# VGLoic/kzg-poly-commit-exploration

Hardware: AMD Instinct MI355X
Metric: g1_msm_commitments_per_sec_degree_2^20 (higher is better)
Workload: dtype i32 digits (Fp: 13 signed radix-2^30 digits, Montgomery 2^390; Fr: 8 x u32, Montgomery 2^256)

## Files before the change

kzg_poly_commit_exploration_amd/csrc/api.hip:

```cpp
#include <hip/hip_runtime.h>
#include <sys/random.h>

#include <algorithm>
#include <atomic>
#include <cerrno>
#include <chrono>
#include <condition_variable>
#include <cstdio>
#include <cstdlib>
#include <cstring>
#include <deque>
#include <functional>
#include <mutex>
#include <new>
#include <string>
#include <thread>
#include <vector>

#include "../../include/kzg_mi355x.h"
#include "engine.h"
#include "host_field.hpp"
#include "host_fr.hpp"
#include "fr30_host.hpp"
#include "host_pairing.hpp"
#include "host_sha256.hpp"
#include "wire30.hip.h"

using namespace kzg;
namespace hf = kzg_host;

namespace {

constexpr size_t kMaxCoefficients = 0xFFFFFFFFull;

#ifndef KZG_NUM_SLOTS
#define KZG_NUM_SLOTS 5
#endif
constexpr int kNumSlots = KZG_NUM_SLOTS;
struct ReducePlan {
    uint32_t lo_bits = 0, hi_bits = 0;
    uint32_t row_lo = 0, row_hi = 0;
    uint32_t col_lo = 0, col_hi = 0;
    uint32_t off_r2row = 0, off_c2row = 0, off_r2col = 0, off_c2col = 0, total = 0;
};

enum SlotKind { SLOT_IDLE = 0, SLOT_COMMIT = 1, SLOT_OPEN = 2, SLOT_TRIVIAL = 3, SLOT_COMMIT_BATCH = 4, SLOT_OPEN_BATCH = 5, SLOT_RESERVED = 6,
                SLOT_OPEN_POINTS = 7 ,
                SLOT_OPEN_COMBINED = 8 ,
                SLOT_OPEN_SETS = 9  };

int hip_fail(kzg_ctx* ctx, const char* what, hipError_t e);

struct DevBuf {
    void* p = nullptr;
    size_t cap = 0;
    DevBuf() = default;
    DevBuf(const DevBuf&) = delete;
    DevBuf& operator=(const DevBuf&) = delete;
    ~DevBuf() { reset(); }
    void reset() {
        if (p) hipFree(p);
        p = nullptr;
        cap = 0;
    }
    template <class T = uint32_t> T* dev() const { return (T*)p; }
    int reserve(kzg_ctx* ctx, size_t bytes, hipStream_t drain = nullptr) { return bytes <= cap ? KZG_OK : grow(ctx, bytes, drain); }
    int grow(kzg_ctx* ctx, size_t bytes, hipStream_t drain) {
        if (drain)
            if (hipError_t e = hipStreamSynchronize(drain)) return hip_fail(ctx, "hipStreamSynchronize", e);
        reset();
        if (hipError_t e = hipMalloc(&p, bytes)) {
            p = nullptr;
            return hip_fail(ctx, "hipMalloc", e);
        }
        cap = bytes;
        return KZG_OK;
    }
};
struct PinnedBuf {
    enum Kind { Mapped, Staged };
    const Kind kind;
    void *h = nullptr, *d = nullptr;
    size_t cap = 0;
    explicit PinnedBuf(Kind k) : kind(k) {}
    PinnedBuf(const PinnedBuf&) = delete;
    PinnedBuf& operator=(const PinnedBuf&) = delete;
    ~PinnedBuf() { reset(); }
    void reset() {
        if (h) hipHostFree(h);
        if (d && kind == Staged) hipFree(d);
        h = d = nullptr;
        cap = 0;
    }
    template <class T = uint32_t> T* host() const { return (T*)h; }
    template <class T = uint32_t> T* dev() const { return (T*)d; }
    int reserve(kzg_ctx* ctx, size_t bytes, hipStream_t drain = nullptr) { return bytes <= cap ? KZG_OK : grow(ctx, bytes, drain); }
    int grow(kzg_ctx* ctx, size_t bytes, hipStream_t drain) {
        if (drain)
            if (hipError_t e = hipStreamSynchronize(drain)) return hip_fail(ctx, "hipStreamSynchronize", e);
        reset();
        hipError_t e = hipHostMalloc(&h, bytes, kind == Mapped ? hipHostMallocMapped : hipHostMallocDefault);
        if (e == hipSuccess) e = kind == Mapped ? hipHostGetDevicePointer(&d, h, 0) : hipMalloc(&d, bytes);
        if (e != hipSuccess) {
            d = nullptr;
            reset();
            return hip_fail(ctx, kind == Mapped ? "hipHostMalloc (mapped)" : "hipHostMalloc + hipMalloc (staging)", e);
        }
        cap = bytes;
        return KZG_OK;
    }
};
template <int N>
struct Workspace {
    DevBuf buf[N];
    int get(kzg_ctx* ctx, int i, size_t bytes, void** out) {
        DevBuf& b = buf[i];
        int rc = KZG_OK;
        if (!bytes && !b.p) {
            rc = b.reserve(ctx, 256);
            b.cap = 0;
        } else {
            rc = b.reserve(ctx, bytes);
        }
        *out = b.p;
        return rc;
    }
};

struct SlotQueue {
    hipStream_t stream = nullptr;
    hipStream_t end = nullptr;
    hipEvent_t ev[8] = {};
    hipEvent_t done = nullptr;
    hipEvent_t sorted_ev = nullptr, accum_ev = nullptr;
    hipEvent_t cmb_ev[2] = {};
    hipEvent_t cells_ev = nullptr;
    hipEvent_t upload_ev = nullptr;
    SlotQueue() = default;
    SlotQueue(const SlotQueue&) = delete;
    SlotQueue& operator=(const SlotQueue&) = delete;
    ~SlotQueue() {
        for (hipEvent_t e : {ev[0], ev[1], ev[2], ev[3], ev[4], ev[5], ev[6], ev[7], cmb_ev[0], cmb_ev[1], cells_ev, upload_ev, done, sorted_ev, accum_ev})
            if (e) hipEventDestroy(e);
    }
};

struct Slot : SlotQueue {
    DevBuf cnt, offs, block_sums, pairs, sorted, buckets;
    DevBuf recoded;
    DevBuf part_a, part_b;
    DevBuf pair_scratch;
    DevBuf heavy_ws;
    DevBuf arena;
    PinnedBuf fin{PinnedBuf::Mapped};
    DevBuf stage;
    DevBuf q;
    DevBuf chunk, block;
    PinnedBuf small{PinnedBuf::Mapped};
    PinnedBuf bsmall{PinnedBuf::Mapped};
    std::vector<uint32_t> open_ys;
    PinnedBuf roots{PinnedBuf::Staged};
    PinnedBuf pvals{PinnedBuf::Mapped};
    DevBuf pblock;
    std::vector<uint32_t> pts_ys;
    size_t pts_nq = 0;
    PinnedBuf ctab{PinnedBuf::Staged};
    PinnedBuf cvals{PinnedBuf::Mapped};
    DevBuf cpart, cin;
    size_t cmb_t = 0;
    float combine_ms = 0;
    PinnedBuf stab{PinnedBuf::Staged}, ssel{PinnedBuf::Staged};
    PinnedBuf svals{PinnedBuf::Mapped};
    DevBuf sg;
    std::vector<uint32_t> sets_vmap;
    PinnedBuf ltab{PinnedBuf::Staged};
    DevBuf lag_part;
    DevBuf gp_in, gp_z, gp_part;
    PinnedBuf gp_flags{PinnedBuf::Mapped};
    DevBuf cpoly, cagg;
    SlotKind kind = SLOT_IDLE;
    size_t job_n = 0;
    uint32_t job_batch = 1;
    uint32_t open_y[8] = {};
    bool timing = false;
    bool has_quotient = false;
    bool tail_checked = false;
    kzg_kernel_times times = {};
};

}

struct kzg_ctx {
    kzg::MultiState* multi = nullptr;
    int device = 0;
    std::mutex mu;
    std::condition_variable slot_cv;
    int sync_owned = 0;
    bool raw_partials = false;
    bool host_trace = false;
    std::atomic<uint64_t> trace_ns[5] = {};
    std::atomic<uint64_t> trace_calls{0};
    std::string last_error;
    size_t n = 0;
    MsmConfig cfg = {};
    DevBuf table;
    DevBuf ntt_tw;
    DevBuf lag_table;
    size_t lag_n = 0;
    uint64_t srs_gen = 0;
    ReducePlan plan;
    size_t arena_records = 0, final_records = 0;
    uint32_t max_batch = 1;
    Slot slots[kNumSlots];
    hipStream_t front_stream = nullptr, heavy_stream = nullptr, tail_stream = nullptr;
    hipStream_t upload_stream = nullptr;
    uint32_t accum_lds_bytes = 41u * 1024u;
    uint32_t small_lds_bytes = 48u * 1024u;
    bool small_msm_off = false;
    bool slots_ready = false;
    bool timing = false;
    std::mutex fk20_mu;
    DevBuf glv;
    uint32_t glv_log = 0;
    DevBuf fk20_B, fk20_tab;
    uint32_t fk20_log_L = 0, fk20_log_l = 0;
    Workspace<11> fk20_ws;
    std::mutex recover_mu;
    DevBuf rec_g;
    Workspace<11> rec_ws;
    Workspace<17> vc_ws;
    Workspace<8> blob_ws;
    std::mutex lookup_mu;
    Workspace<6> lu_ws;
    std::mutex quotient_mu;
    Workspace<11> pq_ws;
    uint32_t pq_zinv_key = ~0u;
    std::vector<kzg_circuit*> circuits;
};

struct kzg_circuit {
    kzg_ctx* owner = nullptr;
    uint32_t lg_n = 0, lg_ext = 0;
    size_t n = 0, t = 0;
    uint64_t shifts[4 * kPqMaxColumns] = {};
    DevBuf values;
    DevBuf coeffs;
    DevBuf coset;
    DevBuf l0;
    DevBuf zinv;
    size_t N() const { return n << lg_ext; }
    size_t cols() const { return 2 * t + 2; }
};

namespace {

#define HIP_TRY(ctx, expr)                                                                          \
    do {                                                                                            \
        hipError_t _e = (expr);                                                                     \
        if (_e != hipSuccess) {                                                                     \
            (ctx)->last_error = std::string(#expr) + ": " + hipGetErrorString(_e);                  \
            return KZG_ERR_HIP;                                                                     \
        }                                                                                           \
    } while (0)

int hip_fail(kzg_ctx* ctx, const char* what, hipError_t e) {
// ... 47 lines not shown
    if (!ctx->upload_stream) HIP_TRY(ctx, hipStreamCreateWithFlags(&ctx->upload_stream, hipStreamNonBlocking));
    for (auto& e : s.ev)
        if (!e) HIP_TRY(ctx, hipEventCreate(&e));
    if (!s.upload_ev) HIP_TRY(ctx, hipEventCreateWithFlags(&s.upload_ev, hipEventDisableTiming));
    s.stream = s.end = ctx->front_stream;
    if (!s.done) HIP_TRY(ctx, hipEventCreateWithFlags(&s.done, hipEventDisableTiming));
    return s.small.reserve(ctx, 64 * 4);
}

int upload_unlocked(kzg_ctx* ctx, std::unique_lock<std::mutex>& lk, Slot& s, void* dst, const void* src, size_t bytes) {
    if (!bytes) return KZG_OK;
    int rc = copy_unlocked(ctx, lk, ctx->upload_stream, dst, src, bytes, hipMemcpyHostToDevice, kCopyCoeffs);
    if (rc) return rc;
    HIP_TRY(ctx, hipEventRecord(s.upload_ev, ctx->upload_stream));
    HIP_TRY(ctx, hipStreamWaitEvent(s.stream, s.upload_ev, 0));
    return KZG_OK;
}

int ensure_poly(kzg_ctx* ctx, Slot& s, size_t n) {
    const size_t cap = n < 1024 ? 1024 : n;
    if (cap * 32 <= s.stage.cap) return KZG_OK;
    if (s.done) HIP_TRY(ctx, hipEventSynchronize(s.done));
    HIP_TRY(ctx, hipStreamSynchronize(ctx->upload_stream));
    HIP_TRY(ctx, hipStreamSynchronize(s.stream));
    for (DevBuf* b : {&s.stage, &s.q, &s.chunk, &s.block}) b->reset();
    int rc = s.stage.reserve(ctx, cap * 32);
    if (rc == KZG_OK) rc = s.q.reserve(ctx, cap * 32);
    if (rc == KZG_OK) rc = s.chunk.reserve(ctx, poly_chunk_words((uint32_t)cap) * 4);
    if (rc == KZG_OK) rc = s.block.reserve(ctx, poly_block_words((uint32_t)cap) * 4);
    if (rc) s.stage.reset();
    return rc;
}

void plan_reduce(kzg_ctx* ctx) {
    ReducePlan P;
    uint32_t bits = 0;
    while ((1u << bits) < ctx->cfg.nb) bits++;
    P.lo_bits = bits / 2;
    P.hi_bits = bits - P.lo_bits;
    P.row_lo = P.hi_bits / 2;
    P.row_hi = P.hi_bits - P.row_lo;
    P.col_lo = P.lo_bits / 2;
    P.col_hi = P.lo_bits - P.col_lo;
    P.off_r2row = 0;
    P.off_c2row = P.off_r2row + (1u << P.row_hi);
    P.off_r2col = P.off_c2row + (1u << P.row_lo);
    P.off_c2col = P.off_r2col + (1u << P.col_hi);
    P.total = P.off_c2col + (1u << P.col_lo);
    ctx->plan = P;
    ctx->arena_records = ((size_t)1 << P.hi_bits) + ((size_t)1 << P.lo_bits);
    ctx->final_records = P.total;
}

int setup_slots_impl(kzg_ctx* ctx);
int setup_slots(kzg_ctx* ctx, bool keep_table_on_failure = false) {
    ctx->slots_ready = false;
    int rc = setup_slots_impl(ctx);
    if (rc != KZG_OK) {
        for (auto& s : ctx->slots) free_slot_msm(s);
        if (keep_table_on_failure) return rc;
        ctx->table.reset();
        ctx->lag_table.reset();
        ctx->lag_n = 0;
        ctx->n = 0;
        (void)hipGetLastError();
    }
    return rc;
}
int setup_slots_impl(kzg_ctx* ctx) {
    plan_reduce(ctx);
    if (const char* v = std::getenv("KZG_TEST_FAIL_SLOT_ALLOC")) {
        const int mode = std::atoi(v);
        if (mode == 1 || (mode == 2 && ctx->max_batch > 1)) {
            ctx->last_error = "injected allocation failure (KZG_TEST_FAIL_SLOT_ALLOC)";
            return KZG_ERR_HIP;
        }
    }
    if (!ctx->heavy_stream) {
        int rc = create_stream(ctx, &ctx->heavy_stream, true);
        if (rc) return rc;
    }
    if (!ctx->tail_stream) {
        int rc = create_stream(ctx, &ctx->tail_stream, false);
        if (rc) return rc;
    }
    const MsmConfig cfg = ctx->cfg;
    if (ctx->max_batch > sort_max_batch(cfg)) ctx->max_batch = sort_max_batch(cfg);
    const size_t B = ctx->max_batch;
    const size_t pairs = (size_t)cfg.max_digits * ctx->n * B;
    for (int i = 0; i < kNumSlots; i++) {
        Slot& s = ctx->slots[i];
        {
            int rcb = ensure_slot_basics(ctx, s);
            if (rcb) return rcb;
        }
        if (!s.sorted_ev) {
            HIP_TRY(ctx, hipEventCreateWithFlags(&s.sorted_ev, hipEventDisableTiming));
            HIP_TRY(ctx, hipEventCreateWithFlags(&s.accum_ev, hipEventDisableTiming));
        }
        free_slot_msm(s);
        int rc = s.cnt.reserve(ctx, (size_t)sort_count_entries((uint32_t)B, cfg) * 4 + 64);
        if (rc == KZG_OK) rc = s.offs.reserve(ctx, ((size_t)cfg.nb * B + 1) * 4);
        if (rc == KZG_OK) rc = s.block_sums.reserve(ctx, (size_t)sort_workspace_words() * 4);
        if (rc) return rc;
        HIP_TRY(ctx, hipMemset(s.block_sums.p, 0, (size_t)sort_workspace_zero_words() * 4));
        rc = s.pairs.reserve(ctx, (pairs ? pairs : 1) * 8);
        if (rc == KZG_OK) rc = s.recoded.reserve(ctx, (ctx->n * B ? ctx->n * B : 1) * 32);
        if (rc == KZG_OK) rc = s.sorted.reserve(ctx, (pairs ? pairs : 1) * 4);
        if (rc == KZG_OK) rc = s.buckets.reserve(ctx, (size_t)cfg.nb * B * kXyzzBytes);
        if (rc == KZG_OK) rc = s.part_a.reserve(ctx, (size_t)kMaxAccumLanes * kXyzzBytes);
        if (rc == KZG_OK) rc = s.part_b.reserve(ctx, (size_t)kMaxAccumLanes * kXyzzBytes);
        if (rc == KZG_OK) rc = s.pair_scratch.reserve(ctx, accumulate_pair_scratch_bytes(pairs));
        if (rc == KZG_OK) rc = s.heavy_ws.reserve(ctx, heavy_workspace_bytes());
        if (rc == KZG_OK) rc = s.arena.reserve(ctx, ctx->arena_records * B * kXyzzBytes);
        if (rc == KZG_OK) rc = s.fin.reserve(ctx, ctx->final_records * B * kXyzzBytes);
        if (rc) return rc;
        s.kind = SLOT_IDLE;
    }
    ctx->slots_ready = true;
    return KZG_OK;
}

int build_tables(kzg_ctx* ctx, hipStream_t st, void* d_xyzz_tmp, void* d_prefix) {
    const size_t n = ctx->n;
    for (uint32_t j = 1; j < ctx->cfg.W; j++) {
        char* prev = (char*)ctx->table.p + (size_t)(j - 1) * n * kAffineBytes;
        char* next = (char*)ctx->table.p + (size_t)j * n * kAffineBytes;
        launch_table_window(st, prev, (uint32_t)n, ctx->cfg.level_bits, d_xyzz_tmp, d_prefix, next);
    }
    HIP_TRY(ctx, hipGetLastError());
    HIP_TRY(ctx, hipStreamSynchronize(st));
    return KZG_OK;
}

int drain_all(kzg_ctx* ctx) {
    for (hipStream_t st : {ctx->upload_stream, ctx->front_stream, ctx->heavy_stream, ctx->tail_stream})
        if (st) HIP_TRY(ctx, hipStreamSynchronize(st));
    return KZG_OK;
}

static int srs_release(kzg_ctx* ctx) {
    ctx->slots_ready = false;
    int rc = drain_all(ctx);
    if (rc) return rc;
    for (auto& s : ctx->slots) s.kind = SLOT_IDLE;
    ctx->table.reset();
    ctx->fk20_B.reset();
    ctx->fk20_tab.reset();
    ctx->lag_table.reset();
    ctx->lag_n = 0;
    ctx->srs_gen++;
    ctx->n = 0;
    return KZG_OK;
}

int srs_prepare(kzg_ctx* ctx, size_t n) {
    if (n == 0 || n > 0x7fffffffu / 32) return KZG_ERR_INVALID_ARG;
    int rc = srs_release(ctx);
    if (rc) return rc;
    size_t free_b = 0, total_b = 0;
    HIP_TRY(ctx, hipMemGetInfo(&free_b, &total_b));
    size_t budget = (size_t)((double)free_b * 0.6);
    if (const char* v = std::getenv("KZG_TABLE_GB")) budget = (size_t)(std::strtod(v, nullptr) * 1073741824.0);
    MsmConfig cfg = choose_msm_config(n, budget);
    if ((size_t)cfg.W * n >= 0x80000000ull) return KZG_ERR_INVALID_ARG;
    ctx->cfg = cfg;
    return ctx->table.reserve(ctx, (size_t)cfg.W * n * kAffineBytes);
}

struct MsmBasis {
    const void* table;
    uint32_t stride;
};
int enqueue_msm(kzg_ctx* ctx, Slot& s, const uint32_t* d_scalars, int is_mont, size_t n, int ev_base,
                uint32_t batch = 1, uint64_t stride = 0, const MsmBasis* basis = nullptr) {
    const MsmConfig cfg = ctx->cfg;
    const void* table = basis ? basis->table : ctx->table.p;
    const uint32_t table_stride = basis ? basis->stride : (uint32_t)ctx->n;
    const uint32_t nbt = cfg.nb * batch;
    hipStream_t st = s.stream;
    s.end = st;
    if (s.timing) HIP_TRY(ctx, hipEventRecord(s.ev[ev_base], st));
    const bool header_zeroed = launch_bucket_sort(st, d_scalars, is_mont, (uint32_t)n, batch, stride, table_stride, cfg, s.cnt.dev(),
                       s.block_sums.dev(), s.pairs.dev<uint64_t>(), s.recoded.dev(), s.offs.dev(), s.sorted.dev(), (uint32_t*)s.heavy_ws.p);
    if (s.timing) {
        HIP_TRY(ctx, hipEventRecord(s.ev[ev_base + 1], st));
        HIP_TRY(ctx, hipEventRecord(s.ev[ev_base + 2], st));
    }
    bool alone = true;
    for (const auto& other : ctx->slots) alone = alone && (&other == &s || other.kind == SLOT_IDLE);
    const uint64_t max_refs = (uint64_t)n * cfg.max_digits * batch;
    const uint32_t lanes = accumulate_lanes(max_refs, alone);
    const ReducePlan& P = ctx->plan;
    const uint32_t R = 1u << P.hi_bits, C = 1u << P.lo_bits, B = batch;
    char* row = (char*)s.arena.p;
    char* col = row + (size_t)R * B * kXyzzBytes;
    char* fin = (char*)s.fin.d;
    const uint32_t rl = 1u << P.row_lo, rh = 1u << P.row_hi, cl = 1u << P.col_lo, ch = 1u << P.col_hi;
    const TreeSumDesc stage1[2] = {
        {s.buckets.p, row, B * R, C, C, 1, B * R, 0},
        {s.buckets.p, col, B * C, R, 1, C, C, (uint64_t)cfg.nb}};
    const TreeSumDesc stage2[4] = {
        {row, fin + (size_t)P.off_r2row * B * kXyzzBytes, B * rh, rl, rl, 1, rh, R},
        {row, fin + (size_t)P.off_c2row * B * kXyzzBytes, B * rl, rh, 1, rl, rl, R},
        {col, fin + (size_t)P.off_r2col * B * kXyzzBytes, B * ch, cl, cl, 1, ch, C},
        {col, fin + (size_t)P.off_c2col * B * kXyzzBytes, B * cl, ch, 1, cl, cl, C}};
    if (!header_zeroed) HIP_TRY(ctx, hipMemsetAsync(s.heavy_ws.p, 0, kHeavyHeaderBytes, st));
    if (max_refs <= kTinyRefs && !ctx->small_msm_off) {
        if (s.timing) HIP_TRY(ctx, hipEventRecord(s.ev[ev_base + 3], st));
        launch_small_msm(st, table, s.sorted.dev(), s.offs.dev(), nbt, lanes, max_refs, s.buckets.p, s.part_a.p, s.part_b.p,
                         s.heavy_ws.p, s.small.dev() + 26, stage1, stage2, ctx->small_lds_bytes);
        if (s.timing) HIP_TRY(ctx, hipEventRecord(s.ev[ev_base + 4], st));
    } else {
        const bool hand_over = !alone;
        hipStream_t hs = hand_over ? ctx->heavy_stream : st;
        if (hand_over) {
            HIP_TRY(ctx, hipEventRecord(s.sorted_ev, st));
            HIP_TRY(ctx, hipStreamWaitEvent(hs, s.sorted_ev, 0));
        }
        if (s.timing) HIP_TRY(ctx, hipEventRecord(s.ev[ev_base + 3], hs));
        launch_bucket_accumulate(hs, table, s.sorted.dev(), s.offs.dev(), nbt, lanes, s.buckets.p, s.part_a.p, s.part_b.p,
                                 ctx->accum_lds_bytes, s.pair_scratch.p, max_refs,
                                 (char*)s.heavy_ws.p + kAccumClockOffset);
        if (s.timing) HIP_TRY(ctx, hipEventRecord(s.ev[ev_base + 4], hs));
        if (hand_over) {
            HIP_TRY(ctx, hipEventRecord(s.accum_ev, hs));
            st = s.end = ctx->tail_stream;
            HIP_TRY(ctx, hipStreamWaitEvent(st, s.accum_ev, 0));
        }
        launch_bucket_finalize(st, s.offs.dev(), nbt, lanes, s.part_a.p, s.part_b.p, s.buckets.p, s.heavy_ws.p, s.small.dev() + 26,
                               finalize_group_size(nbt));
        launch_tree_sums_two_stage(st, stage1, 2, stage2, 4, (uint32_t*)s.heavy_ws.p + 64, alone);
    }
    if (s.timing) HIP_TRY(ctx, hipEventRecord(s.ev[ev_base + 5], st));
    HIP_TRY(ctx, hipGetLastError());
    return KZG_OK;
}

hf::PX host_wsum(const uint64_t* recs, uint32_t len) {
    hf::PX run = hf::px_inf(), acc = hf::px_inf();
    for (uint32_t v = len; v-- > 1;) {
        run = hf::px_add(run, hf::px_from_record(recs + (size_t)v * kXyzzWords64));
        acc = hf::px_add(acc, run);
    }
    return acc;
}
hf::PX host_shift(hf::PX p, uint32_t k) {
    for (uint32_t i = 0; i < k; i++) p = hf::px_double(p);
    return p;
}
hf::P1 finish_msm(const kzg_ctx* ctx, const Slot& s, uint32_t p = 0, uint32_t batch = 1) {
    const ReducePlan& P = ctx->plan;
    const uint64_t* f = s.fin.host<uint64_t>();
    auto at = [&](uint32_t off, uint32_t len) { return f + ((size_t)off * batch + (size_t)p * len) * kXyzzWords64; };
    const uint32_t rh = 1u << P.row_hi, rl = 1u << P.row_lo, ch = 1u << P.col_hi, cl = 1u << P.col_lo;
    hf::PX w_row = hf::px_add(host_shift(host_wsum(at(P.off_r2row, rh), rh), P.row_lo), host_wsum(at(P.off_c2row, rl), rl));
    hf::PX w_col = hf::px_add(host_shift(host_wsum(at(P.off_r2col, ch), ch), P.col_lo), host_wsum(at(P.off_c2col, cl), cl));
    hf::PX total = hf::px_add(host_shift(w_row, P.lo_bits), w_col);
    if (ctx->cfg.recode == kRecodeNaf) total = hf::px_double(total);
    const uint64_t* r2 = at(P.off_r2row, rh);
    for (uint32_t k = 0; k < rh; k++) total = hf::px_add(total, hf::px_from_record(r2 + (size_t)k * kXyzzWords64));
    return ctx->raw_partials ? hf::px_to_jacobian(total) : hf::px_normalize(total);
}

void write_p1(uint64_t out[18], const hf::P1& p) { std::memcpy(out, &p, sizeof p); }

void fill_device_times(Slot& s) {
    s.times.references = s.small.host()[26];
    const uint64_t not_start = (uint64_t)s.small.host()[28] | ((uint64_t)s.small.host()[29] << 32);
    const uint64_t end = (uint64_t)s.small.host()[30] | ((uint64_t)s.small.host()[31] << 32);
    if (not_start != 0 && end > ~not_start) s.times.accumulate_ms = (float)((double)(end - ~not_start) * 1e-5);
}
void fill_accumulate_times(Slot& s) {
    float ms = 0;
    (void)hipEventElapsedTime(&ms, s.ev[3], s.ev[4]);
    s.times.accumulate_events_ms = ms;
    if (s.times.accumulate_ms == 0) s.times.accumulate_ms = ms;
}

void slot_idle(kzg_ctx* ctx, Slot& s) {
    s.kind = SLOT_IDLE;
    ctx->slot_cv.notify_all();
}
int reserve_slot(kzg_ctx* ctx, std::unique_lock<std::mutex>& lk, bool block) {
    for (;;) {
        for (int i = 0; i < kNumSlots; i++)
            if (ctx->slots[i].kind == SLOT_IDLE) {
                ctx->slots[i].kind = SLOT_RESERVED;
                ctx->sync_owned++;
                return i;
            }
        if (!block || ctx->sync_owned == 0) return -1;
        ctx->slot_cv.wait(lk);
    }
}
void release_owned(kzg_ctx* ctx, int slot) {
    if (ctx->slots[slot].kind == SLOT_RESERVED) ctx->slots[slot].kind = SLOT_IDLE;
    ctx->sync_owned--;
    ctx->slot_cv.notify_all();
}
struct SlotLease {
    kzg_ctx* ctx;
    int slot;
    ~SlotLease() { if (slot >= 0) release_owned(ctx, slot); }
};
void quiesce(kzg_ctx* ctx, std::unique_lock<std::mutex>& lk) {
    while (ctx->sync_owned > 0) ctx->slot_cv.wait(lk);
}

bool host_tail_nonzero(const uint64_t* coeffs, size_t from, size_t n) {
    for (size_t i = from; i < n; i++)
        if (coeffs[4 * i] | coeffs[4 * i + 1] | coeffs[4 * i + 2] | coeffs[4 * i + 3]) return true;
    return false;
}

int points_weights(kzg_ctx* ctx, const uint64_t* zs, size_t k, uint64_t* ws ) {
    if (k < 1 || k > KZG_MAX_OPEN_POINTS) {
        ctx->last_error = "multiproof: k must be in [1, KZG_MAX_OPEN_POINTS]";
        return KZG_ERR_INVALID_ARG;
    }
// ... 60 lines not shown
    switch (status) {
        case KZG_OK: return "ok";
        case KZG_ERR_DEGREE_TOO_HIGH:
            return "Setup does not allow for commitment generation of the polynomial. The polynomial degree is too high.";
        case KZG_ERR_CONSTANT_POLY: return "Unable to divide a constant polynomial";
        case KZG_ERR_REMAINDER:
            return "[divide_by_root] Fail to divide the polynomial by a root, constant terms do not add up";
        case KZG_ERR_INVALID_ARG: return "invalid argument";
        case KZG_ERR_NO_DEVICE: return "no HIP device available (this library has no CPU path)";
        case KZG_ERR_HIP: return "HIP runtime error";
        case KZG_ERR_NO_SRS: return "no SRS loaded";
        case KZG_ERR_BUSY: return "slot busy";
        default: return "unknown status";
    }
}

const char* kzg_last_error(const kzg_ctx* ctx) {
    if (!ctx) return "";
    if (ctx->multi && ctx->last_error.empty()) return multi_last_error(ctx->multi);
    return ctx->last_error.c_str();
}

int kzg_ctx_create_multi_ex(const int* devices, int ndev, unsigned flags, kzg_ctx** out) {
    if (!out) return KZG_ERR_INVALID_ARG;
    *out = nullptr;
    if (!devices || ndev <= 0 || (flags & ~(unsigned)KZG_MULTI_REPLICATE_SRS)) return KZG_ERR_INVALID_ARG;
    kzg::MultiState* m = nullptr;
    std::string err;
    int rc = multi_create(devices, ndev, (flags & KZG_MULTI_REPLICATE_SRS) ? kMultiReplicate : kMultiRange, &m, err);
    if (rc != KZG_OK) return rc;
    kzg_ctx* ctx = new kzg_ctx();
    ctx->multi = m;
    ctx->device = devices[0];
    *out = ctx;
    return KZG_OK;
}
int kzg_ctx_create_multi(const int* devices, int ndev, kzg_ctx** out) { return kzg_ctx_create_multi_ex(devices, ndev, 0u, out); }
int kzg_abi_version(void) { return KZG_ABI_VERSION; }
int kzg_num_devices(const kzg_ctx* ctx) { return !ctx ? 0 : (ctx->multi ? multi_num_devices(ctx->multi) : 1); }
uint64_t kzg_rccl_exchanges(const kzg_ctx* ctx) { return (ctx && ctx->multi) ? multi_rccl_exchanges(ctx->multi) : 0; }

int kzg_ctx_create(int device, kzg_ctx** out) {
    if (!out) return KZG_ERR_INVALID_ARG;
    *out = nullptr;
    int count = 0;
    if (hipGetDeviceCount(&count) != hipSuccess || count <= 0) return KZG_ERR_NO_DEVICE;
    if (device < 0 || device >= count) return KZG_ERR_NO_DEVICE;
    if (hipSetDevice(device) != hipSuccess) return KZG_ERR_NO_DEVICE;
    kzg_ctx* ctx = new kzg_ctx();
    ctx->device = device;
    if (const char* v = std::getenv("KZG_ACCUM_LDS_KB")) ctx->accum_lds_bytes = (uint32_t)std::atoi(v) * 1024u;
    if (const char* v = std::getenv("KZG_SMALL_MSM")) ctx->small_msm_off = std::atoi(v) == 0;
    if (const char* v = std::getenv("KZG_HOST_TRACE")) ctx->host_trace = std::atoi(v) != 0;
    if (hipFuncSetAttribute(small_msm_kernel(), hipFuncAttributeMaxDynamicSharedMemorySize, (int)small_msm_lds_bytes()) == hipSuccess)
        ctx->small_lds_bytes = small_msm_lds_bytes();
    else
        (void)hipGetLastError();
    if (!poly_prepare_device() || !points_prepare_device() || !sets_prepare_device()) {
        delete ctx;
        return KZG_ERR_HIP;
    }
    *out = ctx;
    return KZG_OK;
}

void kzg_ctx_destroy(kzg_ctx* ctx) {
    if (!ctx) return;
    if (ctx->multi) {
        multi_destroy(ctx->multi);
        delete ctx;
        return;
    }
    hipSetDevice(ctx->device);
    if (ctx->host_trace && ctx->trace_calls.load()) {
        const double k = 1e-3 / (double)ctx->trace_calls.load();
        std::fprintf(stderr, "[kzg host trace] %llu kzg_commit calls, us per call: wait-for-slot %.1f upload %.1f submit %.1f device %.1f collect %.1f\n",
                     (unsigned long long)ctx->trace_calls.load(), k * ctx->trace_ns[0].load(), k * ctx->trace_ns[1].load(),
                     k * ctx->trace_ns[2].load(), k * ctx->trace_ns[3].load(), k * ctx->trace_ns[4].load());
    }
    for (hipStream_t st : {ctx->upload_stream, ctx->front_stream, ctx->heavy_stream, ctx->tail_stream})
        if (st) hipStreamSynchronize(st);
    for (hipStream_t st : {ctx->upload_stream, ctx->front_stream, ctx->heavy_stream, ctx->tail_stream})
        if (st) hipStreamDestroy(st);
    for (kzg_circuit* c : ctx->circuits) delete c;
    delete ctx;
}

size_t kzg_srs_len(const kzg_ctx* ctx) { return !ctx ? 0 : (ctx->multi ? multi_srs_len(ctx->multi) : ctx->n); }
int kzg_num_slots(const kzg_ctx*) { return kNumSlots; }

int kzg_msm_config(const kzg_ctx* ctx, int* digit_bits, int* table_levels, size_t* num_buckets, int* recoding) {
    if (ctx && ctx->multi)
        return kzg_msm_config(multi_kid(ctx->multi, 0), digit_bits, table_levels, num_buckets, recoding);
    if (!ctx || !ctx->n) return KZG_ERR_NO_SRS;
    if (digit_bits) *digit_bits = (int)ctx->cfg.c;
    if (table_levels) *table_levels = (int)ctx->cfg.W;
    if (num_buckets) *num_buckets = ctx->cfg.nb;
    if (recoding) *recoding = (int)ctx->cfg.recode;
    return KZG_OK;
}

int kzg_srs_load_g1(kzg_ctx* ctx, const void* first_g1, size_t stride, size_t n) {
    if (!ctx || !first_g1 || stride < 144) return KZG_ERR_INVALID_ARG;
    if (ctx->multi) {
        std::lock_guard<std::mutex> lkm(ctx->mu);
        ctx->last_error.clear();
// ... 509 lines not shown
        const std::string why = ctx->last_error;
        ctx->max_batch = previous;
        (void)hipGetLastError();
        (void)setup_slots(ctx);
        ctx->last_error = why;
    }
    return rc;
}

size_t kzg_max_batch(const kzg_ctx* ctx) {
    if (ctx && ctx->multi) return kzg_max_batch(multi_kid(ctx->multi, 0));
    return ctx ? ctx->max_batch : 0;
}

static int commit_batch_submit_locked(kzg_ctx* ctx, int slot, const void* d_coeffs, size_t n, size_t batch,
                                      size_t stride_coeffs, bool owned = false, bool lagrange = false) {
    if (!ctx->n || !ctx->slots_ready) return KZG_ERR_NO_SRS;
    MsmBasis basis{};
    if (lagrange && !lagrange_basis(ctx, n, &basis)) return KZG_ERR_NO_SRS;
    if (slot < 0 || slot >= kNumSlots || batch > ctx->max_batch) return KZG_ERR_INVALID_ARG;
    if (n > ctx->n) return KZG_ERR_DEGREE_TOO_HIGH;
    Slot& s = ctx->slots[slot];
    if (s.kind != (owned ? SLOT_RESERVED : SLOT_IDLE)) return KZG_ERR_BUSY;
    HIP_TRY(ctx, hipSetDevice(ctx->device));
    s.timing = ctx->timing;
    s.end = s.stream;
    s.has_quotient = false;
    s.job_n = n;
    s.job_batch = (uint32_t)batch;
    s.tail_checked = true;
    std::memset(&s.times, 0, sizeof s.times);
    std::memset(s.small.host(), 0, 64 * 4);
    int rc = enqueue_msm(ctx, s, (const uint32_t*)d_coeffs, 1, n, 0, (uint32_t)batch, stride_coeffs, lagrange ? &basis : nullptr);
    if (rc) return rc;
    HIP_TRY(ctx, hipEventRecord(s.done, s.end));
    s.kind = SLOT_COMMIT_BATCH;
    return KZG_OK;
}

int kzg_commit_batch_submit(kzg_ctx* ctx, int slot, const void* d_coeffs, size_t n, size_t batch,
                            size_t stride_coeffs) {
    KZG_SINGLE_DEVICE_ONLY(ctx);
    if (!ctx || !d_coeffs || n == 0 || batch == 0 || stride_coeffs < n || n > kMaxCoefficients) return KZG_ERR_INVALID_ARG;
    std::lock_guard<std::mutex> lk(ctx->mu);
    return commit_batch_submit_locked(ctx, slot, d_coeffs, n, batch, stride_coeffs);
}

static int wait_batch_locked(kzg_ctx* ctx, int slot, uint64_t* out_p1s, size_t batch, size_t out_stride = 18) {
    if (slot < 0 || slot >= kNumSlots) return KZG_ERR_INVALID_ARG;
    Slot& s = ctx->slots[slot];
    if (s.kind != SLOT_COMMIT_BATCH || s.job_batch != batch) return KZG_ERR_INVALID_ARG;
    HIP_TRY(ctx, hipSetDevice(ctx->device));
    slot_idle(ctx, s);
    HIP_TRY(ctx, hipEventSynchronize(s.done));
    fill_device_times(s);
    if (s.timing) {
        float ms = 0;
        (void)hipEventElapsedTime(&ms, s.ev[0], s.ev[1]); s.times.digits_ms = ms;
        (void)hipEventElapsedTime(&ms, s.ev[2], s.ev[3]); s.times.scatter_ms = ms;
        fill_accumulate_times(s);
        (void)hipEventElapsedTime(&ms, s.ev[4], s.ev[5]); s.times.reduce_ms = ms;
        (void)hipEventElapsedTime(&ms, s.ev[0], s.ev[5]); s.times.total_ms = ms;
    }
    const uint32_t B = s.job_batch;
    const uint32_t nthreads = B <= 2 ? 1 : (B < 8 ? B : 8);
    auto work = [&](uint32_t t) {
        for (uint32_t p = t; p < B; p += nthreads) write_p1(out_p1s + out_stride * (size_t)p, finish_msm(ctx, s, p, B));
    };
    if (nthreads <= 1) {
        work(0);
    } else {
        std::vector<std::thread> pool;
        for (uint32_t t = 1; t < nthreads; t++) pool.emplace_back(work, t);
        work(0);
        for (auto& th : pool) th.join();
    }
    return KZG_OK;
}

int kzg_wait_batch(kzg_ctx* ctx, int slot, uint64_t* out_p1s, size_t batch) {
    KZG_SINGLE_DEVICE_ONLY(ctx);
    if (!ctx || !out_p1s) return KZG_ERR_INVALID_ARG;
    std::lock_guard<std::mutex> lk(ctx->mu);
    return wait_batch_locked(ctx, slot, out_p1s, batch);
}

static int open_batch_submit_locked(kzg_ctx* ctx, int slot, const void* d_coeffs, size_t n, size_t batch, size_t stride_coeffs,
                                    const uint64_t* zs, const uint64_t* ys, bool owned = false) {
    if (!ctx->n || !ctx->slots_ready) return KZG_ERR_NO_SRS;
    if (slot < 0 || slot >= kNumSlots || batch > ctx->max_batch) return KZG_ERR_INVALID_ARG;
    if (n - 1 > ctx->n) return KZG_ERR_DEGREE_TOO_HIGH;
    Slot& s = ctx->slots[slot];
    if (s.kind != (owned ? SLOT_RESERVED : SLOT_IDLE)) return KZG_ERR_BUSY;
    HIP_TRY(ctx, hipSetDevice(ctx->device));
    int rc = owned ? KZG_OK : ensure_poly(ctx, s, n * batch);
    if (rc == KZG_OK) rc = s.bsmall.reserve(ctx, batch * 32 * 4, s.stream);
    if (rc) return rc;
    s.timing = ctx->timing;
    s.end = s.stream;
    s.job_n = n;
    s.job_batch = (uint32_t)batch;
    s.has_quotient = true;
    s.tail_checked = true;
    s.open_ys.assign((const uint32_t*)ys, (const uint32_t*)ys + 8 * batch);
    std::memset(&s.times, 0, sizeof s.times);
    std::memset(s.small.host(), 0, 64 * 4);
    std::memset(s.bsmall.host(), 0, batch * 32 * 4);
    if (s.timing) HIP_TRY(ctx, hipEventRecord(s.ev[6], s.stream));
    const size_t nq = n - 1;
    for (size_t p = 0; p < batch; p++) {
        const uint32_t* cp = (const uint32_t*)d_coeffs + p * stride_coeffs * 8;
        uint32_t zw[8];
        std::memcpy(zw, zs + 4 * p, 32);
        uint32_t* sm = s.bsmall.dev() + p * 32;
        PolyScratch sc{s.chunk.dev(), s.block.dev(), sm, sm + 8};
        launch_quotient(s.stream, cp, (uint32_t)n, zw, s.q.dev() + p * nq * 8, sc);
    }
    if (s.timing) HIP_TRY(ctx, hipEventRecord(s.ev[7], s.stream));
    rc = enqueue_msm(ctx, s, s.q.dev(), 1, nq, 0, (uint32_t)batch, nq);
    if (rc) return rc;
    HIP_TRY(ctx, hipEventRecord(s.done, s.end));
    s.kind = SLOT_OPEN_BATCH;
    return KZG_OK;
}

int kzg_open_batch_submit(kzg_ctx* ctx, int slot, const void* d_coeffs, size_t n, size_t batch, size_t stride_coeffs,
                          const uint64_t* zs, const uint64_t* ys) {
    KZG_SINGLE_DEVICE_ONLY(ctx);
    if (!ctx || !d_coeffs || !zs || !ys || n < 2 || batch == 0 || stride_coeffs < n || n > kMaxCoefficients) return KZG_ERR_INVALID_ARG;
    std::lock_guard<std::mutex> lk(ctx->mu);
    return open_batch_submit_locked(ctx, slot, d_coeffs, n, batch, stride_coeffs, zs, ys);
}

static int wait_open_batch_locked(kzg_ctx* ctx, int slot, uint64_t* out_p1s, int* statuses, size_t batch, size_t out_stride = 18,
                                  size_t status_stride = 1) {
    if (slot < 0 || slot >= kNumSlots) return KZG_ERR_INVALID_ARG;
    Slot& s = ctx->slots[slot];
    if (s.kind != SLOT_OPEN_BATCH || s.job_batch != batch || s.open_ys.size() != 8 * batch)
        return KZG_ERR_INVALID_ARG;
    HIP_TRY(ctx, hipSetDevice(ctx->device));
    slot_idle(ctx, s);
    HIP_TRY(ctx, hipEventSynchronize(s.done));
    fill_device_times(s);
    if (s.timing) {
        float ms = 0;
        (void)hipEventElapsedTime(&ms, s.ev[6], s.ev[7]); s.times.quotient_ms = ms;
        (void)hipEventElapsedTime(&ms, s.ev[0], s.ev[1]); s.times.digits_ms = ms;
        fill_accumulate_times(s);
        (void)hipEventElapsedTime(&ms, s.ev[4], s.ev[5]); s.times.reduce_ms = ms;
        (void)hipEventElapsedTime(&ms, s.ev[6], s.ev[5]); s.times.total_ms = ms;
    }
    const uint32_t B = s.job_batch;
    const hf::P1 inf = hf::p1_inf();
    for (uint32_t p = 0; p < B; p++) {
        const uint32_t* hs = s.bsmall.host() + p * 32;
        const uint32_t* y = s.open_ys.data() + 8 * p;
        uint64_t* out = out_p1s + out_stride * (size_t)p;
        int& status = statuses[status_stride * (size_t)p];
        if (!(hs[0] & 1u)) {
            if (std::memcmp(hs + 16, y, 32) != 0) status = KZG_ERR_CONSTANT_POLY;
            else { status = KZG_OK; write_p1(out, inf); }
            continue;
        }
        if (std::memcmp(hs + 8, y, 32) != 0) { status = KZG_ERR_REMAINDER; continue; }
        status = KZG_OK;
        write_p1(out, finish_msm(ctx, s, p, B));
    }
    s.open_ys.clear();
    return KZG_OK;
}

int kzg_wait_open_batch(kzg_ctx* ctx, int slot, uint64_t* out_p1s, int* statuses, size_t batch) {
    KZG_SINGLE_DEVICE_ONLY(ctx);
    if (!ctx || !out_p1s || !statuses) return KZG_ERR_INVALID_ARG;
    std::lock_guard<std::mutex> lk(ctx->mu);
    return wait_open_batch_locked(ctx, slot, out_p1s, statuses, batch);
}

int kzg_wait(kzg_ctx* ctx, int slot, uint64_t out_p1[18]) {
    KZG_SINGLE_DEVICE_ONLY(ctx);
    if (!ctx || !out_p1) return KZG_ERR_INVALID_ARG;
    std::lock_guard<std::mutex> lk(ctx->mu);
    return wait_locked(ctx, slot, out_p1);
}


static void await_unlocked(std::unique_lock<std::mutex>& lk, Slot& s) {
    if (s.kind == SLOT_TRIVIAL || s.kind == SLOT_RESERVED || s.kind == SLOT_IDLE) return;
    lk.unlock();
    (void)hipEventSynchronize(s.done);
    lk.lock();
}

struct HostTrace {
    kzg_ctx* ctx;
    std::chrono::steady_clock::time_point t;
    explicit HostTrace(kzg_ctx* c) : ctx(c) { if (c->host_trace) t = std::chrono::steady_clock::now(); }
    void mark(int phase) {
        if (!ctx->host_trace) return;
        const auto now = std::chrono::steady_clock::now();
        ctx->trace_ns[phase] += (uint64_t)std::chrono::duration_cast<std::chrono::nanoseconds>(now - t).count();
        t = now;
    }
};

static int commit_host(kzg_ctx* ctx, const void* scalars, int is_mont, size_t n, uint64_t out_p1[18]) {
    if (!ctx || !out_p1 || (!scalars && n)) return KZG_ERR_INVALID_ARG;
    if (n > kMaxCoefficients) return KZG_ERR_INVALID_ARG;
    if (ctx->multi) return multi_commit(ctx->multi, scalars, is_mont, n, out_p1);
    HostTrace tr(ctx);
    std::unique_lock<std::mutex> lk(ctx->mu);
    if (!ctx->n || !ctx->slots_ready) return KZG_ERR_NO_SRS;
    HIP_TRY(ctx, hipSetDevice(ctx->device));
    if (n > ctx->n && host_tail_nonzero((const uint64_t*)scalars, ctx->n, n)) return KZG_ERR_DEGREE_TOO_HIGH;
    const int slot = reserve_slot(ctx, lk, true);
    if (slot < 0) return KZG_ERR_BUSY;
    Slot& s = ctx->slots[slot];
    const size_t n_dev = n < ctx->n ? n : ctx->n;
    int rc = ensure_poly(ctx, s, n_dev);
    tr.mark(0);
// ... 6287 lines not shown
```

Before: 439.8.

## Split large batched MSMs into per-polynomial pipelined sort/accumulate/reduce stages

For batched commitments whose per-polynomial reference count exceeds a threshold, each polynomial is sorted, accumulated and reduced as its own sub-job. The sub-jobs run across the front, heavy and tail streams with per-polynomial events, so one polynomial's sort can overlap another's accumulation and reduction. The host finishes each result as soon as its tail event fires instead of waiting for the whole batch. This costs extra workspace (per-polynomial heavy workspaces and up to four sets of partial buffers), more events and launches, and per-polynomial finalize launches.

```diff
diff --git a/kzg_poly_commit_exploration_amd/csrc/api.hip b/kzg_poly_commit_exploration_amd/csrc/api.hip
--- a/kzg_poly_commit_exploration_amd/csrc/api.hip
+++ b/kzg_poly_commit_exploration_amd/csrc/api.hip
@@ -37,6 +37,9 @@
 #define KZG_NUM_SLOTS 5
 #endif
 constexpr int kNumSlots = KZG_NUM_SLOTS;
+constexpr uint64_t kBatchSplitRefs = 12u << 20;
+constexpr uint32_t kSplitMaxBatch = 32;
+constexpr uint32_t kSplitPartSets = 4;
 struct ReducePlan {
     uint32_t lo_bits = 0, hi_bits = 0;
     uint32_t row_lo = 0, row_hi = 0;
@@ -136,12 +139,14 @@
     hipEvent_t cmb_ev[2] = {};
     hipEvent_t cells_ev = nullptr;
     hipEvent_t upload_ev = nullptr;
+    std::vector<hipEvent_t> sub_ev;
     SlotQueue() = default;
     SlotQueue(const SlotQueue&) = delete;
     SlotQueue& operator=(const SlotQueue&) = delete;
     ~SlotQueue() {
         for (hipEvent_t e : {ev[0], ev[1], ev[2], ev[3], ev[4], ev[5], ev[6], ev[7], cmb_ev[0], cmb_ev[1], cells_ev, upload_ev, done, sorted_ev, accum_ev})
             if (e) hipEventDestroy(e);
+        for (hipEvent_t e : sub_ev) hipEventDestroy(e);
     }
 };
 
@@ -158,6 +163,7 @@
     DevBuf chunk, block;
     PinnedBuf small{PinnedBuf::Mapped};
     PinnedBuf bsmall{PinnedBuf::Mapped};
+    PinnedBuf sub_stats{PinnedBuf::Mapped};
     std::vector<uint32_t> open_ys;
     PinnedBuf roots{PinnedBuf::Staged};
     PinnedBuf pvals{PinnedBuf::Mapped};
@@ -181,6 +187,7 @@
     SlotKind kind = SLOT_IDLE;
     size_t job_n = 0;
     uint32_t job_batch = 1;
+    bool job_split = false;
     uint32_t open_y[8] = {};
     bool timing = false;
     bool has_quotient = false;
@@ -211,6 +218,8 @@
     ReducePlan plan;
     size_t arena_records = 0, final_records = 0;
     uint32_t max_batch = 1;
+    uint64_t split_refs = kBatchSplitRefs;
+    uint32_t split_polys = 1;
     Slot slots[kNumSlots];
     hipStream_t front_stream = nullptr, heavy_stream = nullptr, tail_stream = nullptr;
     hipStream_t upload_stream = nullptr;
@@ -364,6 +373,8 @@
     ctx->final_records = P.total;
 }
 
+size_t heavy_ws_stride() { return (heavy_workspace_bytes() + 255) & ~(size_t)255; }
+
 int setup_slots_impl(kzg_ctx* ctx);
 int setup_slots(kzg_ctx* ctx, bool keep_table_on_failure = false) {
     ctx->slots_ready = false;
@@ -400,6 +411,10 @@
     if (ctx->max_batch > sort_max_batch(cfg)) ctx->max_batch = sort_max_batch(cfg);
     const size_t B = ctx->max_batch;
     const size_t pairs = (size_t)cfg.max_digits * ctx->n * B;
+    const uint64_t poly_refs = (uint64_t)cfg.max_digits * ctx->n;
+    const bool can_split = B > 1 && ctx->split_refs != 0 && poly_refs >= ctx->split_refs && poly_refs > kTinyRefs;
+    ctx->split_polys = can_split ? (uint32_t)std::min<size_t>(B, kSplitMaxBatch) : 1u;
+    const size_t part_sets = std::min(ctx->split_polys, kSplitPartSets);
     for (int i = 0; i < kNumSlots; i++) {
         Slot& s = ctx->slots[i];
         {
@@ -412,7 +427,7 @@
         }
         free_slot_msm(s);
         int rc = s.cnt.reserve(ctx, (size_t)sort_count_entries((uint32_t)B, cfg) * 4 + 64);
-        if (rc == KZG_OK) rc = s.offs.reserve(ctx, ((size_t)cfg.nb * B + 1) * 4);
+        if (rc == KZG_OK) rc = s.offs.reserve(ctx, ((size_t)cfg.nb + 1) * B * 4);
         if (rc == KZG_OK) rc = s.block_sums.reserve(ctx, (size_t)sort_workspace_words() * 4);
         if (rc) return rc;
         HIP_TRY(ctx, hipMemset(s.block_sums.p, 0, (size_t)sort_workspace_zero_words() * 4));
@@ -420,10 +435,10 @@
         if (rc == KZG_OK) rc = s.recoded.reserve(ctx, (ctx->n * B ? ctx->n * B : 1) * 32);
         if (rc == KZG_OK) rc = s.sorted.reserve(ctx, (pairs ? pairs : 1) * 4);
         if (rc == KZG_OK) rc = s.buckets.reserve(ctx, (size_t)cfg.nb * B * kXyzzBytes);
-        if (rc == KZG_OK) rc = s.part_a.reserve(ctx, (size_t)kMaxAccumLanes * kXyzzBytes);
-        if (rc == KZG_OK) rc = s.part_b.reserve(ctx, (size_t)kMaxAccumLanes * kXyzzBytes);
+        if (rc == KZG_OK) rc = s.part_a.reserve(ctx, part_sets * kMaxAccumLanes * kXyzzBytes);
+        if (rc == KZG_OK) rc = s.part_b.reserve(ctx, part_sets * kMaxAccumLanes * kXyzzBytes);
         if (rc == KZG_OK) rc = s.pair_scratch.reserve(ctx, accumulate_pair_scratch_bytes(pairs));
-        if (rc == KZG_OK) rc = s.heavy_ws.reserve(ctx, heavy_workspace_bytes());
+        if (rc == KZG_OK) rc = s.heavy_ws.reserve(ctx, ctx->split_polys * heavy_ws_stride());
         if (rc == KZG_OK) rc = s.arena.reserve(ctx, ctx->arena_records * B * kXyzzBytes);
         if (rc == KZG_OK) rc = s.fin.reserve(ctx, ctx->final_records * B * kXyzzBytes);
         if (rc) return rc;
@@ -484,11 +499,102 @@
     const void* table;
     uint32_t stride;
 };
+bool batch_splits(const kzg_ctx* ctx, size_t n, size_t batch) {
+    const uint64_t poly_refs = (uint64_t)n * ctx->cfg.max_digits;
+    return batch > 1 && batch <= ctx->split_polys && ctx->split_refs != 0 && poly_refs >= ctx->split_refs && poly_refs > kTinyRefs;
+}
+using BeforeSort = std::function<int(uint32_t)>;
+
+int enqueue_msm_split(kzg_ctx* ctx, Slot& s, const uint32_t* d_scalars, int is_mont, size_t n, int ev_base, uint32_t batch,
+                      uint64_t stride, const void* table, uint32_t table_stride, const BeforeSort* before_sort) {
+    const MsmConfig cfg = ctx->cfg;
+    const ReducePlan& P = ctx->plan;
+    while (s.sub_ev.size() < 3 * (size_t)batch) {
+        hipEvent_t e = nullptr;
+        HIP_TRY(ctx, hipEventCreateWithFlags(&e, hipEventDisableTiming));
+        s.sub_ev.push_back(e);
+    }
+    int rc = s.sub_stats.reserve(ctx, (size_t)batch * 8 * 4);
+    if (rc) return rc;
+    std::memset(s.sub_stats.host(), 0, (size_t)batch * 8 * 4);
+    s.job_split = true;
+    const uint64_t poly_refs = (uint64_t)n * cfg.max_digits;
+    const uint32_t lanes = accumulate_lanes(poly_refs, false);
+    const uint32_t R = 1u << P.hi_bits, C = 1u << P.lo_bits, B = batch;
+    const uint32_t rl = 1u << P.row_lo, rh = 1u << P.row_hi, cl = 1u << P.col_lo, ch = 1u << P.col_hi;
+    const size_t part_set_bytes = (size_t)kMaxAccumLanes * kXyzzBytes;
+    hipStream_t front = s.stream, heavy = ctx->heavy_stream, tail = ctx->tail_stream;
+    struct Sub {
+        uint32_t *offs, *sorted, *stats;
+        char *buckets, *heavy_ws, *part_a, *part_b;
+    };
+    auto sub = [&](uint32_t p) {
+        Sub u;
+        u.offs = s.offs.dev() + (size_t)p * (cfg.nb + 1);
+        u.sorted = s.sorted.dev() + (size_t)p * poly_refs;
+        u.stats = s.sub_stats.dev() + (size_t)p * 8;
+        u.buckets = (char*)s.buckets.p + (size_t)p * cfg.nb * kXyzzBytes;
+        u.heavy_ws = (char*)s.heavy_ws.p + (size_t)p * heavy_ws_stride();
+        u.part_a = (char*)s.part_a.p + (p % kSplitPartSets) * part_set_bytes;
+        u.part_b = (char*)s.part_b.p + (p % kSplitPartSets) * part_set_bytes;
+        return u;
+    };
+    for (uint32_t p = 0; p < batch; p++) {
+        const Sub u = sub(p);
+        if (before_sort) {
+            rc = (*before_sort)(p);
+            if (rc) return rc;
+        }
+        if (s.timing && p == 0) HIP_TRY(ctx, hipEventRecord(s.ev[ev_base], front));
+        const bool header_zeroed =
+            launch_bucket_sort(front, d_scalars + (size_t)p * stride * 8, is_mont, (uint32_t)n, 1, 0, table_stride, cfg, s.cnt.dev(),
+                               s.block_sums.dev(), s.pairs.dev<uint64_t>() + (size_t)p * poly_refs, s.recoded.dev() + (size_t)p * n * 8,
+                               u.offs, u.sorted, (uint32_t*)u.heavy_ws);
+        if (!header_zeroed) HIP_TRY(ctx, hipMemsetAsync(u.heavy_ws, 0, kHeavyHeaderBytes, front));
+        if (s.timing && p == 0) {
+            HIP_TRY(ctx, hipEventRecord(s.ev[ev_base + 1], front));
+            HIP_TRY(ctx, hipEventRecord(s.ev[ev_base + 2], front));
+        }
+        HIP_TRY(ctx, hipEventRecord(s.sub_ev[3 * p], front));
+    }
+    for (uint32_t p = 0; p < batch; p++) {
+        const Sub u = sub(p);
+        hipEvent_t accum_ev = s.sub_ev[3 * p + 1], tail_ev = s.sub_ev[3 * p + 2];
+        HIP_TRY(ctx, hipStreamWaitEvent(heavy, s.sub_ev[3 * p], 0));
+        if (p >= kSplitPartSets) HIP_TRY(ctx, hipStreamWaitEvent(heavy, s.sub_ev[3 * (p - kSplitPartSets) + 2], 0));
+        if (s.timing && p == 0) HIP_TRY(ctx, hipEventRecord(s.ev[ev_base + 3], heavy));
+        launch_bucket_accumulate(heavy, table, u.sorted, u.offs, cfg.nb, lanes, u.buckets, u.part_a, u.part_b, ctx->accum_lds_bytes,
+                                 s.pair_scratch.p, poly_refs, u.heavy_ws + kAccumClockOffset);
+        if (s.timing && p == batch - 1) HIP_TRY(ctx, hipEventRecord(s.ev[ev_base + 4], heavy));
+        HIP_TRY(ctx, hipEventRecord(accum_ev, heavy));
+        HIP_TRY(ctx, hipStreamWaitEvent(tail, accum_ev, 0));
+        launch_bucket_finalize(tail, u.offs, cfg.nb, lanes, u.part_a, u.part_b, u.buckets, u.heavy_ws, u.stats, finalize_group_size(cfg.nb));
+        char* row = (char*)s.arena.p + (size_t)p * (R + C) * kXyzzBytes;
+        char* col = row + (size_t)R * kXyzzBytes;
+        char* fin = (char*)s.fin.d;
+        auto section = [&](uint32_t off, uint32_t len) { return fin + ((size_t)off * B + (size_t)p * len) * kXyzzBytes; };
+        const TreeSumDesc stage1[2] = {{u.buckets, row, R, C, C, 1, R, 0}, {u.buckets, col, C, R, 1, C, C, (uint64_t)cfg.nb}};
+        const TreeSumDesc stage2[4] = {{row, section(P.off_r2row, rh), rh, rl, rl, 1, rh, R},
+                                       {row, section(P.off_c2row, rl), rl, rh, 1, rl, rl, R},
+                                       {col, section(P.off_r2col, ch), ch, cl, cl, 1, ch, C},
+                                       {col, section(P.off_c2col, cl), cl, ch, 1, cl, cl, C}};
+        launch_tree_sums_two_stage(tail, stage1, 2, stage2, 4, (uint32_t*)u.heavy_ws + 64, false);
+        HIP_TRY(ctx, hipEventRecord(tail_ev, tail));
+    }
+    s.end = tail;
+    if (s.timing) HIP_TRY(ctx, hipEventRecord(s.ev[ev_base + 5], tail));
+    HIP_TRY(ctx, hipGetLastError());
+    return KZG_OK;
+}
+
 int enqueue_msm(kzg_ctx* ctx, Slot& s, const uint32_t* d_scalars, int is_mont, size_t n, int ev_base,
-                uint32_t batch = 1, uint64_t stride = 0, const MsmBasis* basis = nullptr) {
+                uint32_t batch = 1, uint64_t stride = 0, const MsmBasis* basis = nullptr, const BeforeSort* before_sort = nullptr) {
     const MsmConfig cfg = ctx->cfg;
     const void* table = basis ? basis->table : ctx->table.p;
     const uint32_t table_stride = basis ? basis->stride : (uint32_t)ctx->n;
+    s.job_split = false;
+    if (batch_splits(ctx, n, batch))
+        return enqueue_msm_split(ctx, s, d_scalars, is_mont, n, ev_base, batch, stride, table, table_stride, before_sort);
     const uint32_t nbt = cfg.nb * batch;
     hipStream_t st = s.stream;
     s.end = st;
@@ -578,6 +684,18 @@
 void write_p1(uint64_t out[18], const hf::P1& p) { std::memcpy(out, &p, sizeof p); }
 
 void fill_device_times(Slot& s) {
+    if (s.job_split) {
+        uint64_t refs = 0, ticks = 0;
+        for (uint32_t p = 0; p < s.job_batch; p++) {
+            const uint32_t* w = s.sub_stats.host() + (size_t)p * 8;
+            refs += w[0];
+            const uint64_t not_start = (uint64_t)w[2] | ((uint64_t)w[3] << 32), end = (uint64_t)w[4] | ((uint64_t)w[5] << 32);
+            if (not_start != 0 && end > ~not_start) ticks += end - ~not_start;
+        }
+        s.times.references = refs;
+        s.times.accumulate_ms = (float)((double)ticks * 1e-5);
+        return;
+    }
     s.times.references = s.small.host()[26];
     const uint64_t not_start = (uint64_t)s.small.host()[28] | ((uint64_t)s.small.host()[29] << 32);
     const uint64_t end = (uint64_t)s.small.host()[30] | ((uint64_t)s.small.host()[31] << 32);
@@ -744,6 +862,7 @@
     if (const char* v = std::getenv("KZG_ACCUM_LDS_KB")) ctx->accum_lds_bytes = (uint32_t)std::atoi(v) * 1024u;
     if (const char* v = std::getenv("KZG_SMALL_MSM")) ctx->small_msm_off = std::atoi(v) == 0;
     if (const char* v = std::getenv("KZG_HOST_TRACE")) ctx->host_trace = std::atoi(v) != 0;
+    if (const char* v = std::getenv("KZG_BATCH_SPLIT_REFS")) ctx->split_refs = std::strtoull(v, nullptr, 10);
     if (hipFuncSetAttribute(small_msm_kernel(), hipFuncAttributeMaxDynamicSharedMemorySize, (int)small_msm_lds_bytes()) == hipSuccess)
         ctx->small_lds_bytes = small_msm_lds_bytes();
     else
@@ -1359,6 +1478,11 @@
     if (s.kind != SLOT_COMMIT_BATCH || s.job_batch != batch) return KZG_ERR_INVALID_ARG;
     HIP_TRY(ctx, hipSetDevice(ctx->device));
     slot_idle(ctx, s);
+    if (s.job_split)
+        for (uint32_t p = 0; p < s.job_batch; p++) {
+            HIP_TRY(ctx, hipEventSynchronize(s.sub_ev[3 * p + 2]));
+            write_p1(out_p1s + out_stride * (size_t)p, finish_msm(ctx, s, p, s.job_batch));
+        }
     HIP_TRY(ctx, hipEventSynchronize(s.done));
     fill_device_times(s);
     if (s.timing) {
@@ -1369,6 +1493,7 @@
         (void)hipEventElapsedTime(&ms, s.ev[4], s.ev[5]); s.times.reduce_ms = ms;
         (void)hipEventElapsedTime(&ms, s.ev[0], s.ev[5]); s.times.total_ms = ms;
     }
+    if (s.job_split) return KZG_OK;
     const uint32_t B = s.job_batch;
     const uint32_t nthreads = B <= 2 ? 1 : (B < 8 ? B : 8);
     auto work = [&](uint32_t t) {
@@ -1415,16 +1540,26 @@
     std::memset(s.bsmall.host(), 0, batch * 32 * 4);
     if (s.timing) HIP_TRY(ctx, hipEventRecord(s.ev[6], s.stream));
     const size_t nq = n - 1;
-    for (size_t p = 0; p < batch; p++) {
+    auto quotient = [&](size_t p) {
         const uint32_t* cp = (const uint32_t*)d_coeffs + p * stride_coeffs * 8;
         uint32_t zw[8];
         std::memcpy(zw, zs + 4 * p, 32);
         uint32_t* sm = s.bsmall.dev() + p * 32;
         PolyScratch sc{s.chunk.dev(), s.block.dev(), sm, sm + 8};
         launch_quotient(s.stream, cp, (uint32_t)n, zw, s.q.dev() + p * nq * 8, sc);
-    }
-    if (s.timing) HIP_TRY(ctx, hipEventRecord(s.ev[7], s.stream));
-    rc = enqueue_msm(ctx, s, s.q.dev(), 1, nq, 0, (uint32_t)batch, nq);
+    };
+    if (batch_splits(ctx, nq, batch)) {
+        const BeforeSort before_sort = [&](uint32_t p) -> int {
+            quotient(p);
+            if (s.timing && p + 1 == batch) HIP_TRY(ctx, hipEventRecord(s.ev[7], s.stream));
+            return KZG_OK;
+        };
+        rc = enqueue_msm(ctx, s, s.q.dev(), 1, nq, 0, (uint32_t)batch, nq, nullptr, &before_sort);
+    } else {
+        for (size_t p = 0; p < batch; p++) quotient(p);
+        if (s.timing) HIP_TRY(ctx, hipEventRecord(s.ev[7], s.stream));
+        rc = enqueue_msm(ctx, s, s.q.dev(), 1, nq, 0, (uint32_t)batch, nq);
+    }
     if (rc) return rc;
     HIP_TRY(ctx, hipEventRecord(s.done, s.end));
     s.kind = SLOT_OPEN_BATCH;
@@ -1447,6 +1582,27 @@
         return KZG_ERR_INVALID_ARG;
     HIP_TRY(ctx, hipSetDevice(ctx->device));
     slot_idle(ctx, s);
+    const uint32_t B = s.job_batch;
+    const hf::P1 inf = hf::p1_inf();
+    auto collect = [&](uint32_t p) {
+        const uint32_t* hs = s.bsmall.host() + p * 32;
+        const uint32_t* y = s.open_ys.data() + 8 * p;
+        uint64_t* out = out_p1s + out_stride * (size_t)p;
+        int& status = statuses[status_stride * (size_t)p];
+        if (!(hs[0] & 1u)) {
+            if (std::memcmp(hs + 16, y, 32) != 0) status = KZG_ERR_CONSTANT_POLY;
+            else { status = KZG_OK; write_p1(out, inf); }
+            return;
+        }
+        if (std::memcmp(hs + 8, y, 32) != 0) { status = KZG_ERR_REMAINDER; return; }
+        status = KZG_OK;
+        write_p1(out, finish_msm(ctx, s, p, B));
+    };
+    if (s.job_split)
+        for (uint32_t p = 0; p < B; p++) {
+            HIP_TRY(ctx, hipEventSynchronize(s.sub_ev[3 * p + 2]));
+            collect(p);
+        }
     HIP_TRY(ctx, hipEventSynchronize(s.done));
     fill_device_times(s);
     if (s.timing) {
@@ -1457,22 +1613,8 @@
         (void)hipEventElapsedTime(&ms, s.ev[4], s.ev[5]); s.times.reduce_ms = ms;
         (void)hipEventElapsedTime(&ms, s.ev[6], s.ev[5]); s.times.total_ms = ms;
     }
-    const uint32_t B = s.job_batch;
-    const hf::P1 inf = hf::p1_inf();
-    for (uint32_t p = 0; p < B; p++) {
-        const uint32_t* hs = s.bsmall.host() + p * 32;
-        const uint32_t* y = s.open_ys.data() + 8 * p;
-        uint64_t* out = out_p1s + out_stride * (size_t)p;
-        int& status = statuses[status_stride * (size_t)p];
-        if (!(hs[0] & 1u)) {
-            if (std::memcmp(hs + 16, y, 32) != 0) status = KZG_ERR_CONSTANT_POLY;
-            else { status = KZG_OK; write_p1(out, inf); }
-            continue;
-        }
-        if (std::memcmp(hs + 8, y, 32) != 0) { status = KZG_ERR_REMAINDER; continue; }
-        status = KZG_OK;
-        write_p1(out, finish_msm(ctx, s, p, B));
-    }
+    if (!s.job_split)
+        for (uint32_t p = 0; p < B; p++) collect(p);
     s.open_ys.clear();
     return KZG_OK;
 }
```

Measured after the change: 433.2. -1.5%, worse.
